# jlvdb/yet_another_wizz

Hardware: AMD Instinct MI355X
Metric: candidate pairs/s (higher is better)
Workload: dtype f64

## Files before the change

yet_another_wizz_amd/csrc/yawhip.hip:

```cpp

#include <hip/hip_runtime.h>

#include <algorithm>
#include <atomic>
#include <numeric>
#include <thread>
#include <chrono>
#include <climits>
#include <cmath>
#include <cstdarg>
#include <cstdio>
#include <cstdlib>
#include <cstring>
#include <memory>
#include <new>
#include <string>
#include <system_error>
#include <type_traits>
#include <utility>
#include <functional>
#include <vector>

#include "yawhip.h"
#include "yawhip_random.h"
// ... 202 lines not shown
    for (int d = -2; d <= 2; ++d) {
        const int64_t m = r + d;
        int64_t cnt = 0;
        if (d == 0) {
            cnt = i - off[r];
        } else if (m >= g_lo && m < g_hi) {
            int64_t l = off[m], h = off[m + 1];
            const int64_t base = l;
            if (d < 0) { while (l < h) { const int64_t mid = (l + h) >> 1; if (key[mid] <= ki) l = mid + 1; else h = mid; } }
            else       { while (l < h) { const int64_t mid = (l + h) >> 1; if (key[mid] < ki) l = mid + 1; else h = mid; } }
            cnt = l - base;
        }
        before[d + 2] = cnt;
    }
#pragma unroll
    for (int d = -1; d <= 1; ++d) {
        const int64_t t = r + d + 1 + 2 * g;
        const int64_t dst = off3[t] + before[d + 1] + before[d + 2] + before[d + 3];
        q3[dst] = fx; q3[q3_stride + dst] = fy; q3[2 * q3_stride + dst] = fz;
        idx3[dst] = (int32_t)i;
        if (w3) w3[dst] = wi;
        if (d == 0) pos3[i] = (int32_t)dst;
    }
}

constexpr int EVAL_SLOTS = 256;
constexpr int BUILD_WG = 1024;
constexpr int BUILD_WG_SMALL = 256;
inline int build_wg_for(int64_t n_pot) { return n_pot / 256 <= 4096 ? BUILD_WG_SMALL : BUILD_WG; }
constexpr int BUILD_PREFIX_LDS = 1024;

constexpr int ITEM_SEGS = 8;
__host__ __device__ constexpr int ITEM_SEG_CTR(int seg) { return 12 + 8 * seg; }
__device__ __forceinline__ void append_items(bool keep, const Item &it, unsigned long long work, Item *__restrict__ items,
                                             unsigned long long *__restrict__ counters, unsigned char *__restrict__ kept,
                                             unsigned long long seg_cap = 0) {
    if (keep && kept) kept[it.pot] = 1;
    __shared__ unsigned int s_cnt[BUILD_WG / 64];
    __shared__ unsigned long long s_work[BUILD_WG / 64], s_base;
    const unsigned long long mask = __builtin_amdgcn_ballot_w64(keep);
    const int lane = threadIdx.x & 63, wave = threadIdx.x >> 6;
    for (int off = 32; off > 0; off >>= 1) work += __shfl_down(work, off, 64);
    if (lane == 0) {
        s_cnt[wave] = (unsigned int)__popcll(mask);
        s_work[wave] = work;
    }
    __syncthreads();
    if (threadIdx.x == 0) {
        unsigned int total = 0;
        unsigned long long wsum = 0;
        for (int wv = 0; wv < (int)(blockDim.x >> 6); ++wv) {
            const unsigned int c = s_cnt[wv];
            s_cnt[wv] = total;
            total += c;
            wsum += s_work[wv];
        }
        if (seg_cap) {
            const int seg = (int)(blockIdx.x % ITEM_SEGS);
            s_base = (unsigned long long)seg * seg_cap + (total ? atomicAdd(&counters[ITEM_SEG_CTR(seg)], (unsigned long long)total) : 0ull);
        } else {
            s_base = total ? atomicAdd(&counters[0], (unsigned long long)total) : 0ull;
        }
        if (wsum) atomicAdd(&counters[10 + 8 * (blockIdx.x & (EVAL_SLOTS - 1))], wsum);
    }
    __syncthreads();
    if (keep) items[s_base + s_cnt[wave] + __popcll(mask & ((1ull << lane) - 1ull))] = it;
}

template <bool SWEEP>
__global__ __launch_bounds__(BUILD_WG) void k_build_items(CatView c1, CatView c2, const int32_t *__restrict__ jobs,
                                                     const int64_t *__restrict__ prefix, int n_slots, int n_bins,
                                                     int tile, const double *__restrict__ rwin, int64_t n_pot,
                                                     Item *__restrict__ items, unsigned long long *__restrict__ counters,
                                                     unsigned char *__restrict__ kept) {
    const int64_t pot = (int64_t)blockIdx.x * blockDim.x + threadIdx.x;
    bool keep = false;
    Item it{};
    unsigned long long work = 0;
    if (pot < n_pot) {
        int lo = 0, hi = n_slots;
        while (hi - lo > 1) {
            const int mid = (lo + hi) >> 1;
            if (prefix[mid] <= pot) lo = mid; else hi = mid;
        }
        const int slot = lo, job = slot / n_bins, k = slot - job * n_bins;
        const int p = jobs[2 * job], q = jobs[2 * job + 1];
        const int k1 = c1.nb == 1 ? 0 : k, k2 = c2.nb == 1 ? 0 : k;
        int64_t b0 = c1.off[(int64_t)p * c1.nb + k1], b1 = c1.off[(int64_t)p * c1.nb + k1 + 1];
        const int64_t a_seg1 = c2.off[(int64_t)q * c2.nb + k2 + 1];
        const int64_t a0 = c2.off[(int64_t)q * c2.nb + k2] + (pot - prefix[slot]) * (int64_t)tile;
        const int64_t a1 = a0 + tile < a_seg1 ? a0 + tile : a_seg1;
        if (SWEEP) {
            const double wlo = c2.key[a0] - rwin[k], whi = c2.key[a1 - 1] + rwin[k];
            int64_t l = b0, h = b1;
            while (l < h) {
                const int64_t m = (l + h) >> 1;
                if (c1.key[m] < wlo) l = m + 1; else h = m;
            }
            const int64_t first = l;
            h = b1;
            while (l < h) {
                const int64_t m = (l + h) >> 1;
                if (c1.key[m] <= whi) l = m + 1; else h = m;
            }
            b0 = first;
            b1 = l;
        }
        keep = b1 > b0;
        it.a0 = a0; it.b0[0] = b0; it.na = (int32_t)(a1 - a0); it.nb[0] = (int32_t)(b1 - b0); it.nwin = 1; it.slot = slot; it.pot = (int32_t)pot;
        work = keep ? (unsigned long long)it.na * (unsigned long long)it.nb[0] : 0ull;
    }
    if (SWEEP) {
        append_items(keep, it, work, items, counters, kept);
    } else {
        if (pot < n_pot) items[pot] = it;
        append_items(false, it, work, items, counters, nullptr);
        if (pot == 0) counters[0] = (unsigned long long)n_pot;
    }
}

__global__ __launch_bounds__(BUILD_WG) void k_build_items_strips(const DevTab *__restrict__ tabs, const JobRec *__restrict__ jobs,
                                                            const int64_t *__restrict__ prefix, int n_jobs, int reach,
                                                            int tile, double rwin, double cap_c, double cap_s, int swap,
                                                            int triple, int64_t n_pot,
                                                            Item *__restrict__ items, unsigned long long *__restrict__ counters,
                                                            unsigned char *__restrict__ kept, unsigned long long seg_cap) {
    const int64_t pot = (int64_t)blockIdx.x * blockDim.x + threadIdx.x;
    bool keep = false;
    Item it{};
    unsigned long long work = 0;
    __shared__ int64_t s_prefix[BUILD_PREFIX_LDS];
    __shared__ DevTab s_tabs[6];
    static_assert(sizeof(DevTab) % 8 == 0, "DevTab is copied in 8-byte words");
    for (int e = threadIdx.x; e < (int)(6 * sizeof(DevTab) / 8); e += blockDim.x)
        reinterpret_cast<uint64_t *>(s_tabs)[e] = reinterpret_cast<const uint64_t *>(tabs)[e];
    const bool prefix_in_lds = n_jobs + 1 <= BUILD_PREFIX_LDS;
    if (prefix_in_lds)
        for (int e = threadIdx.x; e <= n_jobs; e += blockDim.x) s_prefix[e] = prefix[e];
    __syncthreads();
    if (pot < n_pot) {
        int lo = 0, hi = n_jobs;
        if (prefix_in_lds) {
            while (hi - lo > 1) {
                const int mid = (lo + hi) >> 1;
                if (s_prefix[mid] <= pot) lo = mid; else hi = mid;
            }
        } else {
            while (hi - lo > 1) {
                const int mid = (lo + hi) >> 1;
                if (prefix[mid] <= pot) lo = mid; else hi = mid;
            }
        }
        const int job = lo;
        const JobRec jr = jobs[job];
        const int o = jr.o & 3;
        it.pad_ = (jr.o >> 2) & 1;
        const DevTab &c1 = s_tabs[swap ? 3 + o : o], &c2 = s_tabs[swap ? o : 3 + o];
        const gf64p key1d = tab_key(c1), key2 = tab_key(c2);
        const gf32p key1f = c1.axis == 0 ? c1.qx : (c1.axis == 1 ? c1.qy : c1.qz);
// ... 1270 lines not shown
                    (void)__hip_atomic_fetch_add((__attribute__((address_space(3))) unsigned int *)(size_t)pend[r], 1u,
                                                 __ATOMIC_RELAXED, __HIP_MEMORY_SCOPE_WORKGROUP);
            }
            if (!WEIGHTED && (stage_no & flush_mask) == flush_mask) flush_counts();
        }
        }
        if constexpr (WEIGHTED) {
            __syncthreads();
            for (int idx = lane; idx < nslots; idx += 64) {
                partials[(int64_t)it.pot * nslots + idx] = (double)hist[idx];
                hist[idx] = HistT(0);
            }
        } else {
            flush_counts();
        }
        nev = wave_sum_lane63(nev);
        if (lane == 63 && nev) atomicAdd(&counters[8 + 8 * (ticket & (EVAL_SLOTS - 1))], (unsigned long long)nev);
    }
}

__global__ void k_item_work(const Item *__restrict__ items, const unsigned long long *__restrict__ counters,
                            int slots_per_job, unsigned long long *__restrict__ job_work) {
    const unsigned long long i = (unsigned long long)blockIdx.x * blockDim.x + threadIdx.x;
    if (i >= counters[0]) return;
    const Item it = items[i];
    unsigned long long streamed = 0;
    for (int w = 0; w < it.nwin; ++w) streamed += (unsigned long long)it.nb[w];
    atomicAdd(&job_work[item_slot(it) / slots_per_job], (unsigned long long)it.na * streamed);
}

constexpr int REDUCE_CHUNK = 32;
__global__ void k_reduce_chunks(const double *__restrict__ partials, const unsigned char *__restrict__ kept,
                                const int64_t *__restrict__ prefix, const int64_t *__restrict__ cprefix, int n_slots,
                                int slab, double *__restrict__ chunk_sums) {
    const int64_t idx = (int64_t)blockIdx.x * blockDim.x + threadIdx.x;
    const int64_t g = idx / slab;
    if (g >= cprefix[n_slots]) return;
    const int e = (int)(idx - g * slab);
    int lo = 0, hi = n_slots;
    while (hi - lo > 1) {
        const int mid = (lo + hi) >> 1;
        if (cprefix[mid] <= g) lo = mid; else hi = mid;
    }
    const int64_t p0 = prefix[lo] + (g - cprefix[lo]) * REDUCE_CHUNK;
    const int64_t p1 = p0 + REDUCE_CHUNK < prefix[lo + 1] ? p0 + REDUCE_CHUNK : prefix[lo + 1];
    double acc = 0.0;
    for (int64_t pot = p0; pot < p1; ++pot)
        if (!kept || kept[pot]) acc += partials[pot * slab + e];
    chunk_sums[idx] = acc;
}

__global__ void k_reduce_slots(const double *__restrict__ chunk_sums, const int64_t *__restrict__ cprefix, int n_slots,
                               int slab, double *__restrict__ out) {
    const int64_t idx = (int64_t)blockIdx.x * blockDim.x + threadIdx.x;
    if (idx >= (int64_t)n_slots * slab) return;
    const int slot = (int)(idx / slab), e = (int)(idx - (int64_t)slot * slab);
    double acc = 0.0;
    for (int64_t g = cprefix[slot]; g < cprefix[slot + 1]; ++g) acc += chunk_sums[g * slab + e];
    out[idx] = acc;
}

template <typename F>
__device__ double numpy_sum_dev(F v, int lo, int n) {
    if (n < 8) {
        double res = 0.0;
        for (int i = 0; i < n; ++i) res += v(lo + i);
        return res;
    }
    if (n <= 128) {
        double r[8];
        for (int j = 0; j < 8; ++j) r[j] = v(lo + j);
        int i = 8;
        for (; i < n - (n % 8); i += 8)
            for (int j = 0; j < 8; ++j) r[j] += v(lo + i + j);
        double res = ((r[0] + r[1]) + (r[2] + r[3])) + ((r[4] + r[5]) + (r[6] + r[7]));
        for (; i < n; ++i) res += v(lo + i);
        return res;
    }
    int n2 = n / 2;
    n2 -= n2 % 8;
    return numpy_sum_dev(v, lo, n2) + numpy_sum_dev(v, lo + n2, n - n2);
}

__global__ void k_combine_scales(const unsigned long long *__restrict__ counts, const double *__restrict__ sums, int weighted,
                                 int64_t n_jobs, int n_bins, int nf, int n_scales, const int32_t *__restrict__ slices,
                                 const double *__restrict__ factors, double *__restrict__ out) {
    const int64_t i = (int64_t)blockIdx.x * blockDim.x + threadIdx.x;
    if (i >= n_jobs * n_bins * n_scales) return;
    const int sc = (int)(i % n_scales), k = (int)((i / n_scales) % n_bins);
    const int64_t j = i / ((int64_t)n_scales * n_bins);
    const int lo = slices[2 * (k * n_scales + sc)], hi = slices[2 * (k * n_scales + sc) + 1];
    const int64_t base = (j * n_bins + k) * (int64_t)nf;
    const double *wk = factors ? factors + (int64_t)k * nf : nullptr;
    auto value = [&](int e) {
        const double v = weighted ? sums[base + e] : (double)counts[base + e];
        return wk ? v * wk[e] : v;
    };
    out[i] = hi > lo ? numpy_sum_dev(value, lo, hi - lo) : 0.0;
}

__global__ void k_scatter_rows(const double *__restrict__ in, const int32_t *__restrict__ row_index, int64_t row, int64_t n,
                               double *__restrict__ out) {
    const int64_t i = (int64_t)blockIdx.x * blockDim.x + threadIdx.x;
    if (i >= n) return;
    const int64_t r = i / row;
    out[(int64_t)row_index[r] * row + (i - r * row)] = in[i];
}

__global__ void k_counts_to_double(const unsigned long long *__restrict__ in, double *__restrict__ out, int64_t n) {
    const int64_t i = (int64_t)blockIdx.x * blockDim.x + threadIdx.x;
    if (i < n) out[i] = (double)in[i];
}

inline DevTab make_tab(const double *x, const double *y, const double *z, const double *w, const int32_t *k, const int64_t *off,
                       const int64_t *vbase, const int64_t *slo, const int64_t *tiles, const TileRec *tile_rec, const RunGrid *grid,
                       int axis, const float *q = nullptr, int64_t q_stride = 0, const int32_t *idx = nullptr) {
    return DevTab{(gf64p)x, (gf64p)y, (gf64p)z, (gf64p)w, (gi32p)k, (gi64p)off, (gi64p)vbase, (gi64p)slo, (gi64p)tiles,
                  tile_rec, grid, (gf32p)q, (gf32p)(q ? q + q_stride : nullptr), (gf32p)(q ? q + 2 * q_stride : nullptr), (gi32p)idx,
                  (gi32p)nullptr, axis, 0};
}

template <typename T>
struct DevBuf {
    T *ptr = nullptr;
    size_t cap = 0;
    hipError_t reserve(size_t n) {
        if (n <= cap) return hipSuccess;
        if (ptr) (void)hipFree(ptr);
        ptr = nullptr;
        cap = 0;
        size_t want = n + n / 4 + 64;
        hipError_t e = hipMalloc(reinterpret_cast<void **>(&ptr), want * sizeof(T));
        if (e == hipSuccess) cap = want;
        return e;
    }
    void release() {
        if (ptr) (void)hipFree(ptr);
        ptr = nullptr;
        cap = 0;
    }
};

struct Arena {
    unsigned char *h = nullptr, *d = nullptr;
    size_t cap = 0;
    hipError_t reserve(size_t n) {
        if (n <= cap) return hipSuccess;
        release();
        const size_t want = n + n / 4 + 4096;
        hipError_t e = hipHostMalloc(reinterpret_cast<void **>(&h), want, hipHostMallocPortable);
        if (e == hipSuccess) e = hipMalloc(reinterpret_cast<void **>(&d), want);
        if (e == hipSuccess) cap = want; else release();
        return e;
    }
    void release() {
        if (h) (void)hipHostFree(h);
        if (d) (void)hipFree(d);
        h = d = nullptr;
        cap = 0;
    }
};
inline size_t align16(size_t n) { return (n + 15) & ~(size_t)15; }

}

struct CallBufs {
    hipEvent_t ev0 = nullptr, ev1 = nullptr, evc0 = nullptr, evc1 = nullptr, ev_done = nullptr;
    DevBuf<Item> d_items;
    unsigned long long *d_ctr = nullptr, *d_counts = nullptr;
    double *d_sums = nullptr;
    DevBuf<double> d_partials;
    DevBuf<double> d_chunk_sums;
    DevBuf<unsigned char> d_kept;
    Arena out;
    Arena comb;
    hipError_t make_events() {
        hipError_t e = hipSuccess;
        for (hipEvent_t *ev : {&ev0, &ev1, &evc0, &evc1, &ev_done})
            if (e == hipSuccess && !*ev) e = hipEventCreate(ev);
        return e;
    }
    void release_all() {
        d_items.release(); d_partials.release(); d_chunk_sums.release(); d_kept.release();
        out.release(); comb.release();
        for (hipEvent_t *ev : {&ev0, &ev1, &evc0, &evc1, &ev_done}) {
            if (*ev) (void)hipEventDestroy(*ev);
            *ev = nullptr;
        }
    }
};
constexpr int MAX_BATCH = 4;
constexpr size_t MAX_PLANS = 16;

namespace {
struct HostPlan;

struct CallKey {
    uint64_t c1_uid = 0, c2_uid = 0, opt_gen = 0, hash = 0;
    int32_t n_jobs = 0, n_bins = 0, n_edges = 0, kernel = 0, n_dev = 0;
    bool want_counts = false, want_sums = false, for_work = false;
    const int32_t *jobs = nullptr;
    const double *t = nullptr;
    std::vector<int32_t> own_jobs;
    std::vector<double> own_t;

    CallKey() = default;
    CallKey(const yawhip_ctx *ctx, const yawhip_catalog *c1, const yawhip_catalog *c2, int32_t n_jobs, const int32_t *jobs,
// ... 943 lines not shown
    if (c->x) (void)hipFree(c->x);
    if (c->y) (void)hipFree(c->y);
    if (c->z) (void)hipFree(c->z);
    if (c->w) (void)hipFree(c->w);
    if (c->off) (void)hipFree(c->off);
    for (int o = 0; o < 3; ++o) {
        c->strips[o].release();
        c->seg[o].release();
    }
    delete c;
    return YAWHIP_OK;
}

int yawhip_catalog_device_bytes(const yawhip_catalog *cat, int64_t *bytes) {
    if (!cat || !bytes) return fail(YAWHIP_ERR_INVALID, "yawhip_catalog_device_bytes: NULL argument");
    *bytes = cat->device_bytes;
    return YAWHIP_OK;
}

}

namespace {

struct CallState {
    std::chrono::steady_clock::time_point wall0;
    bool pending = false;
    int64_t n_out = 0;
    size_t o_ctr = 0, o_counts = 0, o_sums = 0;
    bool want_counts = false, want_sums = false, band_ran = false, run_unweighted = false, run_weighted = false;
    bool segmented = false;
    int64_t cand = 0, abytes = 0, n_pot = 0;
    int launches = 0, kernel = 0, mode = 0, n_orient = 0, band_variant = 0, merged_triples = 0;
    int32_t variant[2] = {0, 0};
};

enum VariantFamily : int32_t { VF_COUNT = 1, VF_MERGED, VF_MERGED_OCC8, VF_BAND, VF_BAND32, VF_BAND32_ONE, VF_BAND32_FINE };
constexpr int32_t variant_code(int32_t family, int R, int cap, bool weighted, int ne = 0, bool merged = false, bool uni = false,
                               bool priv = false, bool filter = false, bool nf1 = false) {
    return family | R << 4 | cap << 8 | (int32_t)weighted << 18 | ne << 19 | (int32_t)merged << 22 | (int32_t)uni << 23 |
           (int32_t)priv << 24 | (int32_t)filter << 25 | (int32_t)nf1 << 26;
}
int32_t merge_variant(int32_t a, int32_t b) { return a == 0 || a == b ? b : (b == 0 ? a : YAWHIP_VARIANT_MIXED); }

std::vector<float> build_thr32(const double *t, int n_bins, int n_edges) {
    auto down = [](double v) { float f = (float)v; if ((double)f > v) f = nextafterf(f, -INFINITY); return f; };
    auto up = [](double v) { float f = (float)v; if ((double)f < v) f = nextafterf(f, INFINITY); return f; };
    auto guard = [](double te) { return BAND32_GUARD_SQRT * std::sqrt(te) + 5e-7 * te + 1e-12; };
    const int tw = thr32_width(n_edges);
    std::vector<float> out((size_t)n_bins * tw, 0.f);
    for (int k = 0; k < n_bins; ++k) {
        const double *tk = t + (size_t)k * n_edges;
        float *row = &out[(size_t)k * tw];
        if (n_edges == 2) {
            const double g0 = guard(tk[0]), g1 = guard(tk[1]);
            const float c = (float)(0.5 * (tk[0] + tk[1]));
            const double cd = (double)c;
            const double fold = 4e-7 * cd;
            const double h_in = (std::min(cd - (tk[0] + g0), (tk[1] - g1) - cd) - fold) * (1.0 - 1e-6);
            const double h_out = (std::max(cd - (tk[0] - g0), (tk[1] + g1) - cd) + fold) * (1.0 + 1e-6);
            row[0] = c;
            row[1] = h_in > 0.0 ? down(h_in) : 0.f;
            row[2] = up(std::max(h_out, 0.0));
            row[3] = 0.f;
        } else {
            for (int e = 0; e < n_edges; ++e) {
                const double g = guard(tk[e]);
// ... 571 lines not shown
        if (cand_plan->key == key) {
            plan = cand_plan;
            break;
        }
    if (!plan) {
        std::unique_ptr<HostPlan> fresh(new (std::nothrow) HostPlan());
        if (!fresh) return fail(YAWHIP_ERR_OOM, "host allocation failed");
        const int rc = make_plan(ctx, c1, c2, n_jobs, jobs, n_bins, n_edges, t, kernel, want_counts, want_sums, job_work != nullptr, *fresh);
        if (rc != YAWHIP_OK) return rc;
        key.keep();
        fresh->key = std::move(key);
        if (ctx->plans.size() >= MAX_PLANS) {
            size_t old = 0;
            for (size_t i = 1; i < ctx->plans.size(); ++i)
                if (ctx->plans[i]->stamp < ctx->plans[old]->stamp) old = i;
            HIP_TRY(hipStreamSynchronize(ctx->stream));
            delete ctx->plans[old];
            ctx->plans[old] = ctx->plans.back();
            ctx->plans.pop_back();
        }
        plan = fresh.release();
        ctx->plans.push_back(plan);
    }
    plan->stamp = ++ctx->plan_clock;
    const HostPlan &P = *plan;
    cs.n_out = P.n_out;
    if (P.empty) return YAWHIP_OK;
    if (P.split) return SPLIT_JOBS;
    if (P.run_weighted) HIP_TRY(ctx->d_partials.reserve((size_t)std::max<int64_t>(P.n_items, 1) * P.slab));
    g_trace.mark("plan");
    const size_t o_ctr = 0, o_counts = align16(N_CTR * sizeof(unsigned long long)),
                 o_sums = o_counts + align16((size_t)P.n_out * sizeof(unsigned long long));
    const size_t out_bytes = o_sums + align16((size_t)P.n_out * sizeof(double));
    HIP_TRY(ctx->out.reserve(out_bytes));
    ctx->d_ctr = reinterpret_cast<unsigned long long *>(ctx->out.d + o_ctr);
    ctx->d_counts = reinterpret_cast<unsigned long long *>(ctx->out.d + o_counts);
    ctx->d_sums = reinterpret_cast<double *>(ctx->out.d + o_sums);
    HIP_TRY(hipMemsetAsync(ctx->out.d, 0, P.n_items > 0 ? o_sums : out_bytes, ctx->stream));

    int launches = 0;
    const int64_t n_pot = P.n_items;
    int64_t n_items = P.n_items;
    unsigned long long seg_cap = 0;
    g_trace.mark("memset");
    HIP_TRY(hipEventRecord(ctx->ev0, ctx->stream));
    if (n_pot > 0) {
        if (n_pot >= (1ll << 31))
            return fail(YAWHIP_ERR_INVALID, "too many work items (%lld) in one job", (long long)n_pot);
        const int bwg = build_wg_for(n_pot);
        const unsigned bgrid = (unsigned)((n_pot + bwg - 1) / bwg);
        if (P.strip_items && (P.band32 || P.band_fine) && !job_work && ctx->item_segments)
            seg_cap = (unsigned long long)((bgrid + ITEM_SEGS - 1) / ITEM_SEGS) * (unsigned long long)bwg;
        HIP_TRY(ctx->d_items.reserve(seg_cap ? (size_t)(seg_cap * ITEM_SEGS) : (size_t)n_pot));
        unsigned char *kept_flags = nullptr;
        if (P.run_weighted && P.sweep) {
            HIP_TRY(ctx->d_kept.reserve((size_t)n_pot));
            HIP_TRY(hipMemsetAsync(ctx->d_kept.ptr, 0, (size_t)n_pot, ctx->stream));
            kept_flags = ctx->d_kept.ptr;
        }
        if (P.strip_items)
            hipLaunchKernelGGL(k_build_items_strips, dim3(bgrid), dim3(bwg), 0, ctx->stream, P.d_tabs,
                               reinterpret_cast<const JobRec *>(P.d_jobs), P.d_prefix, (int)P.n_sjobs,
                               P.triple ? 0 : P.reach, (int)P.tile, P.rwin_max, P.cap_c, P.cap_s, P.swap ? 1 : 0, P.triple ? 1 : 0,
                               n_pot, ctx->d_items.ptr,
                               ctx->d_ctr, kept_flags, seg_cap);
        else if (P.sweep)
            hipLaunchKernelGGL(k_build_items<true>, dim3(bgrid), dim3(bwg), 0, ctx->stream, view_of(c1), view_of(c2),
                               P.d_jobs, P.d_prefix, (int)P.n_pslots, n_bins, (int)P.tile,
                               P.d_rwin, n_pot, ctx->d_items.ptr, ctx->d_ctr, kept_flags);
        else
            hipLaunchKernelGGL(k_build_items<false>, dim3(bgrid), dim3(bwg), 0, ctx->stream, view_of(c1), view_of(c2),
                               P.d_jobs, P.d_prefix, (int)P.n_pslots, n_bins, (int)P.tile, P.d_rwin, n_pot,
                               ctx->d_items.ptr, ctx->d_ctr, nullptr);
        HIP_TRY(hipGetLastError());
        ++launches;
        n_items = n_pot;
        if (P.strip_items && !P.band && n_pot > SYNC_GRID_MIN_ITEMS) {
            HIP_TRY(hipMemcpyAsync(ctx->out.h, ctx->d_ctr, 2 * sizeof(unsigned long long), hipMemcpyDeviceToHost, ctx->stream));
            HIP_TRY(hipStreamSynchronize(ctx->stream));
            n_items = (int64_t)reinterpret_cast<unsigned long long *>(ctx->out.h)[0];
        }
    }
    if (job_work) {
        HIP_TRY(ctx->d_jobwork.reserve((size_t)n_jobs));
        HIP_TRY(hipMemsetAsync(ctx->d_jobwork.ptr, 0, sizeof(unsigned long long) * (size_t)n_jobs, ctx->stream));
        if (n_pot > 0) {
            hipLaunchKernelGGL(k_item_work, dim3((unsigned)((n_pot + 255) / 256)), dim3(256), 0, ctx->stream, ctx->d_items.ptr,
                               ctx->d_ctr, P.merged ? 1 : n_bins, ctx->d_jobwork.ptr);
            HIP_TRY(hipGetLastError());
        }
        HIP_TRY(hipMemcpyAsync(job_work, ctx->d_jobwork.ptr, sizeof(int64_t) * (size_t)n_jobs, hipMemcpyDeviceToHost,
                               ctx->stream));
        HIP_TRY(hipStreamSynchronize(ctx->stream));
        return YAWHIP_OK;
    }
    auto reduce_partials = [&]() -> hipError_t {
        const int64_t n_oslots = P.n_pslots, values = P.slab, n_chunks = P.n_chunks;
        hipError_t er = ctx->d_chunk_sums.reserve((size_t)std::max<int64_t>(n_chunks, 1) * values);
        if (er != hipSuccess) return er;
        const int thr = 256;
        const bool all_kept = !(P.run_weighted && P.sweep);
        if (n_chunks > 0)
            hipLaunchKernelGGL(k_reduce_chunks, dim3((unsigned)((n_chunks * values + thr - 1) / thr)), dim3(thr), 0, ctx->stream,
                               ctx->d_partials.ptr, all_kept ? nullptr : ctx->d_kept.ptr, P.d_prefix, P.d_cprefix,
                               (int)n_oslots, (int)values, ctx->d_chunk_sums.ptr);
        hipLaunchKernelGGL(k_reduce_slots, dim3((unsigned)((n_oslots * values + thr - 1) / thr)), dim3(thr), 0, ctx->stream,
                           ctx->d_chunk_sums.ptr, P.d_cprefix, (int)n_oslots, (int)values, ctx->d_sums);
        return hipGetLastError();
    };
    HIP_TRY(hipEventRecord(ctx->evc0, ctx->stream));
    int64_t grid = P.strip_items && n_pot > 65536 ? n_pot / P.grid_div : n_pot;
    const int batch_log2 = ctx->band_batch_log2 >= 0 ? ctx->band_batch_log2 : 0;
    if (!P.run_weighted) grid = std::max<int64_t>(grid >> batch_log2, 8);
    grid = std::min<int64_t>((grid + 7) & ~7ll, 1ll << 22);
    const dim3 band_grid((unsigned)grid), wave(64);
    int flush_log2 = ctx->flush_log2;
    while (flush_log2 > 0 && ((uint64_t)64 * P.R * 2 * P.cap << flush_log2) >= (1ull << 32)) --flush_log2;
    const unsigned flush_mask = (1u << flush_log2) - 1u;
    const std::pair<int, int> stage{P.R, P.cap};
    const std::pair<bool, bool> rows{P.merged, P.uni};
    auto launch_band32 = [&](bool wgt) -> hipError_t {
        const size_t lds = band32_lds(P.weighted, P.cap, P.lean_bins * P.nf, P.merged && !P.uniform_t ? n_bins : 0, n_edges);
        const bool one_chunk = P.triple || !P.strip_items;
        return pick<Bool<false>, Bool<true>>(wgt, [&](auto w) {
            return pick<Int<4>, Int<3>, Int<2>>(n_edges, [&](auto ne) {
                return pick<Rows<true, false>, Rows<true, true>, Rows<false, true>>(rows, [&](auto r) {
                    return pick<Stage<4, B32_CAP_BIG>, Stage<2, B32_CAP_BIG>, Stage<2, B32_CAP>, Stage<1, B32_CAP>>(stage, [&](auto s) {
                        using S = decltype(s);
                        using M = decltype(r);
                        auto kern = one_chunk ? k_count_band32_one<S::R, S::CAP, w, ne, M::MERGED, M::UNI>
                                              : k_count_band32<S::R, S::CAP, w, ne, M::MERGED, M::UNI>;
                        cs.variant[w] = variant_code(one_chunk ? VF_BAND32_ONE : VF_BAND32, S::R, S::CAP, w, ne, M::MERGED, M::UNI);
                        return launch(kern, band_grid, wave, lds, ctx->stream, P.d_tabs, ctx->d_items.ptr, n_bins, P.d_t,
                                      P.d_thr32, P.d_rwin, P.d_ucap, flush_mask, P.swap ? 1 : 0, ctx->d_counts,
                                      ctx->d_partials.ptr, ctx->d_ctr, seg_cap);
                    });
                });
            });
        });
    };
    auto launch_band64 = [&](bool wgt) -> hipError_t {
        return pick<Bool<false>, Bool<true>>(wgt, [&](auto w) {
            return pick<Int<0>, Int<4>, Int<3>, Int<2>>(P.band_ne, [&](auto ne) {
// ... 54 lines not shown
    auto lds_for = [&](bool w, bool priv) { return lds_fixed + (size_t)P.nf * (priv ? WG : 1) * (w ? 8 : 4); };
    auto launch_plain = [&](bool wgt) -> hipError_t {
        const bool priv = lds_for(wgt, true) <= (size_t)ctx->lds_limit;
        return pick<Bool<true>, Bool<false>>(wgt, [&](auto w) {
            return pick<Bool<false>, Bool<true>>(priv, [&](auto pv) {
                return pick<Bool<false>, Bool<true>>(P.filter, [&](auto f) {
                    return pick<Int<4>, Int<2>, Int<1>>(P.R, [&](auto r) {
                        cs.variant[w] = variant_code(VF_COUNT, r, 0, w, 0, false, false, pv, f);
                        return in_pieces(WG, [&](dim3 g, int64_t base) {
                            return launch(k_count<r, w, pv, f>, g, dim3(WG), lds_for(w, pv), ctx->stream, view_of(c1), view_of(c2),
                                          ctx->d_items.ptr, n_bins, n_edges, P.d_t, P.d_dthr, base, ctx->d_counts,
                                          ctx->d_partials.ptr, ctx->d_ctr);
                        });
                    });
                });
            });
        });
    };
    const bool band_ran = n_items > 0 && P.lean && P.band;
    auto launch_count = [&](bool wgt) {
        if (band_ran) return P.band32 ? launch_band32(wgt) : (P.band_fine ? launch_fine(wgt) : launch_band64(wgt));
        return P.lean ? launch_lean(wgt) : launch_plain(wgt);
    };
    if (n_items > 0 && P.run_unweighted) {
        HIP_TRY(launch_count(false));
        ++launches;
    }
    if (n_items > 0 && P.run_weighted) {
        HIP_TRY(launch_count(true));
        ++launches;
        HIP_TRY(reduce_partials());
        launches += 2;
    }
    HIP_TRY(hipEventRecord(ctx->evc1, ctx->stream));
    if (!P.weighted && want_sums) {
        const int thr = 256;
        hipLaunchKernelGGL(k_counts_to_double, dim3((unsigned)((P.n_out + thr - 1) / thr)), dim3(thr), 0, ctx->stream,
                           ctx->d_counts, ctx->d_sums, P.n_out);
        HIP_TRY(hipGetLastError());
        ++launches;
    }
    HIP_TRY(hipEventRecord(ctx->ev1, ctx->stream));
    const size_t fetch = !fetch_results ? o_counts : (want_sums ? out_bytes : (want_counts ? o_sums : o_counts));
    HIP_TRY(hipMemcpyAsync(ctx->out.h, ctx->out.d, fetch, hipMemcpyDeviceToHost, ctx->stream));
    cs.pending = true;
    cs.o_ctr = o_ctr; cs.o_counts = o_counts; cs.o_sums = o_sums;
    cs.band_ran = band_ran; cs.run_unweighted = P.run_unweighted; cs.run_weighted = P.run_weighted;
    cs.cand = P.cand; cs.abytes = P.abytes; cs.n_pot = n_pot; cs.segmented = seg_cap != 0;
    cs.launches = launches; cs.kernel = P.kernel; cs.mode = P.mode;
    cs.n_orient = P.n_orient;
    cs.band_variant = !band_ran ? 0 : (P.band32 ? 32 : (P.band_fine ? 33 : 64));
    cs.merged_triples = band_ran && P.triple ? 1 : 0;
    g_trace.mark("launched");
    return YAWHIP_OK;
}

template <typename T>
void place_rows(T *out, const T *in, int64_t n_rows, int64_t row, const int32_t *at = nullptr) {
    if (!out) return;
    if (!at) {
        row *= n_rows;
        n_rows = 1;
    }
    for (int64_t r = 0; r < n_rows; ++r) {
        T *dst = out + (size_t)(at ? at[r] : 0) * (size_t)row;
        if (in) memcpy(dst, in + (size_t)r * row, sizeof(T) * (size_t)row);
        else memset(dst, 0, sizeof(T) * (size_t)row);
    }
}

int count_finish(yawhip_ctx *ctx, const CallState &cs, int64_t *fine_counts, double *fine_sums, yawhip_stats *stats,
                 const int32_t *row_index = nullptr, int64_t row_len = 0, bool wait_done = false) {
    if (stats) memset(stats, 0, sizeof *stats);
    const int64_t n_rows = !row_index ? 1 : (row_len > 0 ? cs.n_out / row_len : 0), row = row_index ? row_len : cs.n_out;
    if (!cs.pending) {
        place_rows<int64_t>(fine_counts, nullptr, n_rows, row, row_index);
        place_rows<double>(fine_sums, nullptr, n_rows, row, row_index);
        return YAWHIP_OK;
    }
    g_trace.mark("meanwhile");
    HIP_TRY(hipSetDevice(ctx->device));
    if (ctx->spin_wait) {
        hipError_t qe;
        const auto spin0 = std::chrono::steady_clock::now();
        while ((qe = wait_done ? hipEventQuery(ctx->ev_done) : hipStreamQuery(ctx->stream)) == hipErrorNotReady &&
               std::chrono::steady_clock::now() - spin0 < std::chrono::milliseconds(2))
            __builtin_ia32_pause();
        if (qe == hipErrorNotReady) qe = wait_done ? hipEventSynchronize(ctx->ev_done) : hipStreamSynchronize(ctx->stream);
        HIP_TRY(qe);
    } else {
        HIP_TRY(wait_done ? hipEventSynchronize(ctx->ev_done) : hipStreamSynchronize(ctx->stream));
    }
    g_trace.mark("waited");
    place_rows(fine_counts, reinterpret_cast<const int64_t *>(ctx->out.h + cs.o_counts), n_rows, row, row_index);
    place_rows(fine_sums, reinterpret_cast<const double *>(ctx->out.h + cs.o_sums), n_rows, row, row_index);
    const unsigned long long *ctr = reinterpret_cast<const unsigned long long *>(ctx->out.h + cs.o_ctr);
    g_trace.mark("copied");
    if (stats) {
        float ms = 0.f;
        HIP_TRY(hipEventElapsedTime(&ms, ctx->ev0, ctx->ev1));
        float cms = 0.f;
        HIP_TRY(hipEventElapsedTime(&cms, ctx->evc0, ctx->evc1));
        stats->count_ms = cms;
        stats->candidate_pairs = cs.cand;
        unsigned long long tile_pairs = 0;
        for (int i = 0; i < EVAL_SLOTS; ++i) tile_pairs += ctr[10 + 8 * (size_t)i];
        stats->evaluated_pairs = (int64_t)tile_pairs * ((cs.run_unweighted ? 1 : 0) + (cs.run_weighted ? 1 : 0));
        if (cs.band_ran) {
            unsigned long long ev = 0;
            for (int i = 0; i < EVAL_SLOTS; ++i) ev += ctr[8 + 8 * (size_t)i];
            stats->evaluated_pairs = (int64_t)ev;
        }
        stats->algorithmic_bytes = cs.abytes;
        stats->n_workgroups = cs.n_pot > 0 ? (int64_t)ctr[0] : 0;
        if (cs.segmented && cs.n_pot > 0)
            for (int sg = 0; sg < ITEM_SEGS; ++sg) stats->n_workgroups += (int64_t)ctr[ITEM_SEG_CTR(sg)];
        stats->n_launches = cs.launches;
        stats->kernel_used = cs.kernel;
        stats->layout_mode = cs.mode;
        stats->n_orientations = cs.n_orient;
        stats->band_variant = cs.band_variant;
        stats->merged_triples = cs.merged_triples;
        stats->count_variant = cs.variant[0];
        stats->count_variant_weighted = cs.variant[1];
        if (cs.band_ran)
            for (int i = 0; i < EVAL_SLOTS; ++i) stats->exact_reevaluations += (int64_t)ctr[9 + 8 * (size_t)i];
        stats->kernel_ms = ms;
        stats->total_ms = std::chrono::duration<double, std::milli>(std::chrono::steady_clock::now() - cs.wall0).count();
    }
    g_trace.mark("stats");
    return YAWHIP_OK;
}

void add_stats(yawhip_stats &total, const yawhip_stats &part, bool side_by_side) {
    total.candidate_pairs += part.candidate_pairs;
// ... 182 lines not shown
}

int yawhip_count_pairs_rows_device(yawhip_ctx *ctx, const yawhip_catalog *c1, const yawhip_catalog *c2, int32_t n_jobs,
                                   const int32_t *jobs, int32_t n_bins, int32_t n_edges, const double *t, int32_t kernel,
                                   int64_t n_rows_total, const int32_t *row_index, double **device_rows, yawhip_stats *stats) {
    if (stats) memset(stats, 0, sizeof *stats);
    if (!ctx || !c1 || !c2 || !device_rows) return fail(YAWHIP_ERR_INVALID, "yawhip_count_pairs_rows_device: NULL argument");
    *device_rows = nullptr;
    if (!ctx->peers.empty()) return fail(YAWHIP_ERR_INVALID, "yawhip_count_pairs_rows_device: single-device contexts only");
    const int rc_args = check_call(ctx, c1, c2, n_jobs, jobs, n_bins, n_edges, t);
    if (rc_args != YAWHIP_OK) return rc_args;
    if (n_rows_total < n_jobs || (n_jobs > 0 && !row_index))
        return fail(YAWHIP_ERR_INVALID, "yawhip_count_pairs_rows_device: bad sizes or NULL arrays");
    const int64_t row = (int64_t)n_bins * (n_edges - 1);
    for (int j = 0; j < n_jobs; ++j)
        if (row_index[j] < 0 || row_index[j] >= n_rows_total)
            return fail(YAWHIP_ERR_INVALID, "yawhip_count_pairs_rows_device: row index %d outside [0, %lld)", row_index[j], (long long)n_rows_total);
    HIP_TRY(hipSetDevice(ctx->device));
    const size_t n_full = (size_t)n_rows_total * (size_t)row + 1;
    HIP_TRY(ctx->d_full.reserve(n_full));
    HIP_TRY(ctx->d_rowidx.reserve((size_t)std::max(n_jobs, 1)));
    CallState cs;
    int rc = count_enqueue(ctx, c1, c2, n_jobs, jobs, n_bins, n_edges, t, kernel, false, true, nullptr, cs, false);
    if (rc == SPLIT_JOBS) {
        std::vector<double> rows((size_t)n_jobs * (size_t)row), full(n_full, 0.0);
        rc = run_single(ctx, c1, c2, n_jobs, jobs, n_bins, n_edges, t, kernel, nullptr, rows.data(), stats);
        if (rc != YAWHIP_OK) return rc;
        place_rows(full.data(), (const double *)rows.data(), n_jobs, row, row_index);
        HIP_TRY(hipMemcpy(ctx->d_full.ptr, full.data(), sizeof(double) * n_full, hipMemcpyHostToDevice));
        *device_rows = ctx->d_full.ptr;
        return YAWHIP_OK;
    }
    if (rc != YAWHIP_OK) return rc;
    HIP_TRY(hipMemsetAsync(ctx->d_full.ptr, 0, sizeof(double) * n_full, ctx->stream));
    if (cs.pending && n_jobs > 0) {
        HIP_TRY(hipMemcpyAsync(ctx->d_rowidx.ptr, row_index, sizeof(int32_t) * (size_t)n_jobs, hipMemcpyHostToDevice, ctx->stream));
        const int64_t n = (int64_t)n_jobs * row;
        hipLaunchKernelGGL(k_scatter_rows, dim3((unsigned)((n + 255) / 256)), dim3(256), 0, ctx->stream, ctx->d_sums,
                           ctx->d_rowidx.ptr, row, n, ctx->d_full.ptr);
        HIP_TRY(hipGetLastError());
    }
    rc = count_finish(ctx, cs, nullptr, nullptr, stats);
    if (rc != YAWHIP_OK) return rc;
    *device_rows = ctx->d_full.ptr;
    return YAWHIP_OK;
}

}

namespace {
double numpy_sum(const double *a, int64_t n) {
    if (n < 8) {
        double res = 0.0;
        for (int64_t i = 0; i < n; ++i) res += a[i];
        return res;
    }
    if (n <= 128) {
        double r[8];
        for (int j = 0; j < 8; ++j) r[j] = a[j];
        int64_t i = 8;
        for (; i < n - (n % 8); i += 8)
            for (int j = 0; j < 8; ++j) r[j] += a[i + j];
        double res = ((r[0] + r[1]) + (r[2] + r[3])) + ((r[4] + r[5]) + (r[6] + r[7]));
        for (; i < n; ++i) res += a[i];
        return res;
    }
// ... 16 lines not shown
}

namespace {

struct DenseState {
    CallState cs;
    bool enqueued = false;
    bool device_combine = false;
    bool weighted = false;
    int slot = 0;
    int64_t n_comb = 0;
    size_t h_comb_off = 0;
};

int dense_check(const yawhip_ctx *ctx, const yawhip_dense_request &r, int32_t n_bins, int32_t n_edges, const double *t,
                int32_t n_scales, const int32_t *slices) {
    const int rc = check_call(ctx, r.c1, r.c2, r.n_jobs, r.jobs, n_bins, n_edges, t);
    if (rc != YAWHIP_OK) return rc;
    if (n_scales <= 0 || !slices || !r.dense) return fail(YAWHIP_ERR_INVALID, "yawhip_count_pairs_dense: bad sizes or NULL arrays");
    return YAWHIP_OK;
}

int dense_enqueue(yawhip_ctx *ctx, const yawhip_dense_request &r, int32_t n_bins, int32_t n_edges, const double *t, int32_t kernel,
                  int32_t n_scales, const int32_t *slices, const double *fine_factors, DenseState &ds) {
    const int nf = n_edges - 1;
    ds.weighted = r.c1->w != nullptr || r.c2->w != nullptr;
    ds.slot = ctx->slot;
    ds.device_combine = nf > 1;
    int rc = count_enqueue(ctx, r.c1, r.c2, r.n_jobs, r.jobs, n_bins, n_edges, t, kernel, !ds.weighted, ds.weighted, nullptr, ds.cs,
                           !ds.device_combine);
    if (rc == SPLIT_JOBS) return YAWHIP_OK;
    if (rc != YAWHIP_OK) return rc;
    if (ds.device_combine) {
        ds.n_comb = (int64_t)r.n_jobs * n_bins * n_scales;
        const size_t b_slices = align16(sizeof(int32_t) * 2 * (size_t)n_bins * n_scales);
        const size_t b_fact = fine_factors ? align16(sizeof(double) * (size_t)n_bins * nf) : 0;
        HIP_TRY(ctx->comb.reserve(b_slices + b_fact + sizeof(double) * (size_t)std::max<int64_t>(ds.n_comb, 1)));
        memcpy(ctx->comb.h, slices, sizeof(int32_t) * 2 * (size_t)n_bins * n_scales);
        if (fine_factors) memcpy(ctx->comb.h + b_slices, fine_factors, sizeof(double) * (size_t)n_bins * nf);
        HIP_TRY(hipMemcpyAsync(ctx->comb.d, ctx->comb.h, b_slices + b_fact, hipMemcpyHostToDevice, ctx->stream));
        ds.h_comb_off = b_slices + b_fact;
        double *d_comb = reinterpret_cast<double *>(ctx->comb.d + ds.h_comb_off);
        if (ds.cs.pending && ds.n_comb > 0) {
            hipLaunchKernelGGL(k_combine_scales, dim3((unsigned)((ds.n_comb + 255) / 256)), dim3(256), 0, ctx->stream,
                               ctx->d_counts, ctx->d_sums, ds.weighted ? 1 : 0, (int64_t)r.n_jobs, n_bins, nf, n_scales,
                               reinterpret_cast<const int32_t *>(ctx->comb.d),
                               fine_factors ? reinterpret_cast<const double *>(ctx->comb.d + b_slices) : nullptr, d_comb);
            HIP_TRY(hipGetLastError());
            HIP_TRY(hipMemcpyAsync(ctx->comb.h + ds.h_comb_off, d_comb, sizeof(double) * (size_t)ds.n_comb, hipMemcpyDeviceToHost, ctx->stream));
        }
    }
    HIP_TRY(hipEventRecord(ctx->ev_done, ctx->stream));
    ds.enqueued = true;
    return YAWHIP_OK;
}

void dense_clear(const yawhip_dense_request &r, int32_t n_bins, int32_t n_scales) {
    const size_t P = (size_t)r.c1->n_patches;
    memset(r.dense, 0, sizeof(double) * (size_t)n_scales * (size_t)n_bins * P * P);
}

void dense_scatter(const yawhip_dense_request &r, int32_t n_bins, int32_t n_scales, const int32_t *slices, const double *fine_factors,
                   const double *comb, bool weighted, const int64_t *hc, const double *hs) {
    const int64_t P = r.c1->n_patches;
    const int32_t n_jobs = r.n_jobs;
    const int32_t *jobs = r.jobs;
// ... 334 lines not shown
```

Measured before the change: 29280000 billion.

## Replace result memcpy and events with device tail kernel writing coherent host memory

Replaces the device-to-host memcpy and timing events with a tail kernel that copies the result block straight into coherent pinned host memory, zeroes the counter block for the next call, and publishes a sequence word the host spins on. Timing now comes from device wall-clock stamps instead of events. Memsets are skipped when the block is already clean from the previous call's tail. This is meant to cut per-call launch, memset and copy overhead and the event-based host wait, at the cost of coherent-memory writes from the GPU and more complex state tracking.

```diff
diff --git a/yet_another_wizz_amd/csrc/yawhip.hip b/yet_another_wizz_amd/csrc/yawhip.hip
--- a/yet_another_wizz_amd/csrc/yawhip.hip
+++ b/yet_another_wizz_amd/csrc/yawhip.hip
@@ -258,6 +258,12 @@
 
 constexpr int ITEM_SEGS = 8;
 __host__ __device__ constexpr int ITEM_SEG_CTR(int seg) { return 12 + 8 * seg; }
+constexpr int CTR_T_BUILD = 1, CTR_T_COUNTED = 2, CTR_T_TAIL = 3, CTR_TICKET = 4, CTR_DONE = 6;
+__host__ __device__ constexpr int SEG_EXIT_CTR(int seg) { return ITEM_SEG_CTR(seg) + 1; }
+constexpr double CLOCK_MS = 1.0e-5;
+__device__ __forceinline__ void stamp_start(unsigned long long *__restrict__ counters, int word) {
+    if (blockIdx.x == 0 && threadIdx.x == 0) counters[word] = wall_clock64();
+}
 __device__ __forceinline__ void append_items(bool keep, const Item &it, unsigned long long work, Item *__restrict__ items,
                                              unsigned long long *__restrict__ counters, unsigned char *__restrict__ kept,
                                              unsigned long long seg_cap = 0) {
@@ -291,6 +297,7 @@
     }
     __syncthreads();
     if (keep) items[s_base + s_cnt[wave] + __popcll(mask & ((1ull << lane) - 1ull))] = it;
+    if (threadIdx.x == 0) atomicMax(&counters[SEG_EXIT_CTR((int)(blockIdx.x % ITEM_SEGS))], (unsigned long long)wall_clock64());
 }
 
 template <bool SWEEP>
@@ -299,6 +306,7 @@
                                                      int tile, const double *__restrict__ rwin, int64_t n_pot,
                                                      Item *__restrict__ items, unsigned long long *__restrict__ counters,
                                                      unsigned char *__restrict__ kept) {
+    stamp_start(counters, CTR_T_BUILD);
     const int64_t pot = (int64_t)blockIdx.x * blockDim.x + threadIdx.x;
     bool keep = false;
     Item it{};
@@ -351,6 +359,7 @@
                                                             int triple, int64_t n_pot,
                                                             Item *__restrict__ items, unsigned long long *__restrict__ counters,
                                                             unsigned char *__restrict__ kept, unsigned long long seg_cap) {
+    stamp_start(counters, CTR_T_BUILD);
     const int64_t pot = (int64_t)blockIdx.x * blockDim.x + threadIdx.x;
     bool keep = false;
     Item it{};
@@ -1687,7 +1696,8 @@
 constexpr int REDUCE_CHUNK = 32;
 __global__ void k_reduce_chunks(const double *__restrict__ partials, const unsigned char *__restrict__ kept,
                                 const int64_t *__restrict__ prefix, const int64_t *__restrict__ cprefix, int n_slots,
-                                int slab, double *__restrict__ chunk_sums) {
+                                int slab, double *__restrict__ chunk_sums, unsigned long long *__restrict__ counters) {
+    stamp_start(counters, CTR_T_COUNTED);
     const int64_t idx = (int64_t)blockIdx.x * blockDim.x + threadIdx.x;
     const int64_t g = idx / slab;
     if (g >= cprefix[n_slots]) return;
@@ -1706,7 +1716,8 @@
 }
 
 __global__ void k_reduce_slots(const double *__restrict__ chunk_sums, const int64_t *__restrict__ cprefix, int n_slots,
-                               int slab, double *__restrict__ out) {
+                               int slab, double *__restrict__ out, unsigned long long *__restrict__ stamp) {
+    if (stamp) stamp_start(stamp, CTR_T_COUNTED);
     const int64_t idx = (int64_t)blockIdx.x * blockDim.x + threadIdx.x;
     if (idx >= (int64_t)n_slots * slab) return;
     const int slot = (int)(idx / slab), e = (int)(idx - (int64_t)slot * slab);
@@ -1762,9 +1773,39 @@
     out[(int64_t)row_index[r] * row + (i - r * row)] = in[i];
 }
 
-__global__ void k_counts_to_double(const unsigned long long *__restrict__ in, double *__restrict__ out, int64_t n) {
+__global__ void k_counts_to_double(const unsigned long long *__restrict__ in, double *__restrict__ out, int64_t n,
+                                   unsigned long long *__restrict__ counters) {
+    stamp_start(counters, CTR_T_COUNTED);
     const int64_t i = (int64_t)blockIdx.x * blockDim.x + threadIdx.x;
     if (i < n) out[i] = (double)in[i];
+}
+
+constexpr int TAIL_WG = 256;
+constexpr unsigned TAIL_MAX_GRID = 64;
+__global__ __launch_bounds__(TAIL_WG) void k_call_tail(uint4 *__restrict__ dev, uint4 *__restrict__ host, unsigned n_copy,
+                                                      unsigned n_clean, unsigned long long seq) {
+    const unsigned long long t0 = wall_clock64();
+    static_assert(CTR_T_COUNTED == 2 && CTR_T_TAIL == 3 && CTR_TICKET == 4 && CTR_DONE == 6, "units 1, 2 and 3 of the block");
+    for (unsigned u = blockIdx.x * TAIL_WG + threadIdx.x; u < n_copy; u += gridDim.x * TAIL_WG) {
+        if (u == CTR_TICKET / 2 || u == CTR_DONE / 2) continue;
+        uint4 v = dev[u];
+        if (u == CTR_T_COUNTED / 2) {
+            if ((v.x | v.y) == 0u) { v.x = (unsigned)t0; v.y = (unsigned)(t0 >> 32); }
+            v.z = (unsigned)t0; v.w = (unsigned)(t0 >> 32);
+        }
+        host[u] = v;
+        if (u < n_clean) dev[u] = make_uint4(0u, 0u, 0u, 0u);
+    }
+    __threadfence_system();
+    __syncthreads();
+    if (threadIdx.x == 0) {
+        unsigned *ticket = reinterpret_cast<unsigned *>(dev) + 2 * CTR_TICKET;
+        if (atomicInc(ticket, gridDim.x - 1) == gridDim.x - 1) {
+            __threadfence_system();
+            __hip_atomic_store(reinterpret_cast<unsigned long long *>(host) + CTR_DONE, seq, __ATOMIC_RELEASE,
+                               __HIP_MEMORY_SCOPE_SYSTEM);
+        }
+    }
 }
 
 inline DevTab make_tab(const double *x, const double *y, const double *z, const double *w, const int32_t *k, const int64_t *off,
@@ -1803,7 +1844,7 @@
         if (n <= cap) return hipSuccess;
         release();
         const size_t want = n + n / 4 + 4096;
-        hipError_t e = hipHostMalloc(reinterpret_cast<void **>(&h), want, hipHostMallocPortable);
+        hipError_t e = hipHostMalloc(reinterpret_cast<void **>(&h), want, hipHostMallocPortable | hipHostMallocCoherent);
         if (e == hipSuccess) e = hipMalloc(reinterpret_cast<void **>(&d), want);
         if (e == hipSuccess) cap = want; else release();
         return e;
@@ -1828,6 +1869,9 @@
     DevBuf<double> d_chunk_sums;
     DevBuf<unsigned char> d_kept;
     Arena out;
+    bool dirty = true;
+    size_t zero_upto = 0;
+    uint64_t seq = 0;
     Arena comb;
     hipError_t make_events() {
         hipError_t e = hipSuccess;
@@ -2837,6 +2881,11 @@
     int64_t cand = 0, abytes = 0, n_pot = 0;
     int launches = 0, kernel = 0, mode = 0, n_orient = 0, band_variant = 0, merged_triples = 0;
     int32_t variant[2] = {0, 0};
+    uint64_t seq = 0;
+    bool word_wait = true;
+    bool stamps = false;
+    bool cleaned = false;
+    size_t zero_after = 0;
 };
 
 enum VariantFamily : int32_t { VF_COUNT = 1, VF_MERGED, VF_MERGED_OCC8, VF_BAND, VF_BAND32, VF_BAND32_ONE, VF_BAND32_FINE };
@@ -3474,18 +3523,31 @@
     const size_t o_ctr = 0, o_counts = align16(N_CTR * sizeof(unsigned long long)),
                  o_sums = o_counts + align16((size_t)P.n_out * sizeof(unsigned long long));
     const size_t out_bytes = o_sums + align16((size_t)P.n_out * sizeof(double));
+    const unsigned char *const block_was = ctx->out.d;
     HIP_TRY(ctx->out.reserve(out_bytes));
+    if (ctx->out.d != block_was) {
+        ctx->dirty = true;
+        reinterpret_cast<unsigned long long *>(ctx->out.h)[CTR_DONE] = 0;
+    }
     ctx->d_ctr = reinterpret_cast<unsigned long long *>(ctx->out.d + o_ctr);
     ctx->d_counts = reinterpret_cast<unsigned long long *>(ctx->out.d + o_counts);
     ctx->d_sums = reinterpret_cast<double *>(ctx->out.d + o_sums);
-    HIP_TRY(hipMemsetAsync(ctx->out.d, 0, P.n_items > 0 ? o_sums : out_bytes, ctx->stream));
+    const size_t zero_needed = P.n_items > 0 ? o_sums : out_bytes;
+    if (ctx->dirty) ctx->zero_upto = 0;
+    if (ctx->zero_upto < zero_needed) {
+        HIP_TRY(hipMemsetAsync(ctx->out.d + ctx->zero_upto, 0, zero_needed - ctx->zero_upto, ctx->stream));
+        ctx->zero_upto = zero_needed;
+    }
+    ctx->dirty = true;
+    cs.seq = ++ctx->seq;
+    cs.stamps = P.n_items > 0;
 
     int launches = 0;
     const int64_t n_pot = P.n_items;
     int64_t n_items = P.n_items;
     unsigned long long seg_cap = 0;
     g_trace.mark("memset");
-    HIP_TRY(hipEventRecord(ctx->ev0, ctx->stream));
+    if (!cs.stamps) HIP_TRY(hipEventRecord(ctx->ev0, ctx->stream));
     if (n_pot > 0) {
         if (n_pot >= (1ll << 31))
             return fail(YAWHIP_ERR_INVALID, "too many work items (%lld) in one job", (long long)n_pot);
@@ -3545,12 +3607,13 @@
         if (n_chunks > 0)
             hipLaunchKernelGGL(k_reduce_chunks, dim3((unsigned)((n_chunks * values + thr - 1) / thr)), dim3(thr), 0, ctx->stream,
                                ctx->d_partials.ptr, all_kept ? nullptr : ctx->d_kept.ptr, P.d_prefix, P.d_cprefix,
-                               (int)n_oslots, (int)values, ctx->d_chunk_sums.ptr);
+                               (int)n_oslots, (int)values, ctx->d_chunk_sums.ptr, ctx->d_ctr);
         hipLaunchKernelGGL(k_reduce_slots, dim3((unsigned)((n_oslots * values + thr - 1) / thr)), dim3(thr), 0, ctx->stream,
-                           ctx->d_chunk_sums.ptr, P.d_cprefix, (int)n_oslots, (int)values, ctx->d_sums);
+                           ctx->d_chunk_sums.ptr, P.d_cprefix, (int)n_oslots, (int)values, ctx->d_sums,
+                           n_chunks > 0 ? nullptr : ctx->d_ctr);
         return hipGetLastError();
     };
-    HIP_TRY(hipEventRecord(ctx->evc0, ctx->stream));
+    if (!cs.stamps) HIP_TRY(hipEventRecord(ctx->evc0, ctx->stream));
     int64_t grid = P.strip_items && n_pot > 65536 ? n_pot / P.grid_div : n_pot;
     const int batch_log2 = ctx->band_batch_log2 >= 0 ? ctx->band_batch_log2 : 0;
     if (!P.run_weighted) grid = std::max<int64_t>(grid >> batch_log2, 8);
@@ -3671,17 +3734,29 @@
         HIP_TRY(reduce_partials());
         launches += 2;
     }
-    HIP_TRY(hipEventRecord(ctx->evc1, ctx->stream));
+    if (!cs.stamps) HIP_TRY(hipEventRecord(ctx->evc1, ctx->stream));
     if (!P.weighted && want_sums) {
         const int thr = 256;
         hipLaunchKernelGGL(k_counts_to_double, dim3((unsigned)((P.n_out + thr - 1) / thr)), dim3(thr), 0, ctx->stream,
-                           ctx->d_counts, ctx->d_sums, P.n_out);
+                           ctx->d_counts, ctx->d_sums, P.n_out, ctx->d_ctr);
         HIP_TRY(hipGetLastError());
         ++launches;
     }
-    HIP_TRY(hipEventRecord(ctx->ev1, ctx->stream));
+    if (!cs.stamps) HIP_TRY(hipEventRecord(ctx->ev1, ctx->stream));
     const size_t fetch = !fetch_results ? o_counts : (want_sums ? out_bytes : (want_counts ? o_sums : o_counts));
-    HIP_TRY(hipMemcpyAsync(ctx->out.h, ctx->out.d, fetch, hipMemcpyDeviceToHost, ctx->stream));
+    const size_t clean = std::min(fetch, o_sums);
+    const bool sums_written = P.n_items > 0 && (P.run_weighted || want_sums);
+    cs.cleaned = clean == o_sums;
+    cs.zero_after = sums_written ? o_sums : ctx->zero_upto;
+    const unsigned n_copy = (unsigned)(fetch / 16), n_clean = (unsigned)(clean / 16);
+    static_assert(N_CTR * sizeof(unsigned long long) % 16 == 0 && (CTR_DONE + 2) * sizeof(unsigned long long) <= N_CTR * sizeof(unsigned long long),
+                  "the tail's words lie inside the counter block");
+    if (fetch / 16 > 0xffffffffull) return fail(YAWHIP_ERR_INVALID, "result block too large (%zu bytes)", fetch);
+    hipLaunchKernelGGL(k_call_tail, dim3(std::min((n_copy + TAIL_WG - 1) / TAIL_WG, TAIL_MAX_GRID)), dim3(TAIL_WG), 0, ctx->stream,
+                       reinterpret_cast<uint4 *>(ctx->out.d), reinterpret_cast<uint4 *>(ctx->out.h), n_copy, n_clean,
+                       (unsigned long long)cs.seq);
+    HIP_TRY(hipGetLastError());
+    ++launches;
     cs.pending = true;
     cs.o_ctr = o_ctr; cs.o_counts = o_counts; cs.o_sums = o_sums;
     cs.band_ran = band_ran; cs.run_unweighted = P.run_unweighted; cs.run_weighted = P.run_weighted;
@@ -3720,26 +3795,48 @@
     g_trace.mark("meanwhile");
     HIP_TRY(hipSetDevice(ctx->device));
     if (ctx->spin_wait) {
-        hipError_t qe;
+        const unsigned long long *done_word = reinterpret_cast<const unsigned long long *>(ctx->out.h) + CTR_DONE;
+        auto query = [&]() { return wait_done ? hipEventQuery(ctx->ev_done) : hipStreamQuery(ctx->stream); };
+        hipError_t qe = hipErrorNotReady;
         const auto spin0 = std::chrono::steady_clock::now();
-        while ((qe = wait_done ? hipEventQuery(ctx->ev_done) : hipStreamQuery(ctx->stream)) == hipErrorNotReady &&
-               std::chrono::steady_clock::now() - spin0 < std::chrono::milliseconds(2))
+        do {
+            if (cs.word_wait) {
+                if (__atomic_load_n(done_word, __ATOMIC_ACQUIRE) == cs.seq) qe = hipSuccess;
+            } else {
+                qe = query();
+            }
+            if (qe != hipErrorNotReady) break;
             __builtin_ia32_pause();
+        } while (std::chrono::steady_clock::now() - spin0 < std::chrono::milliseconds(2));
+        if (qe == hipSuccess && cs.word_wait) {
+            const hipError_t late = query();
+            if (late != hipErrorNotReady) qe = late;
+        }
         if (qe == hipErrorNotReady) qe = wait_done ? hipEventSynchronize(ctx->ev_done) : hipStreamSynchronize(ctx->stream);
         HIP_TRY(qe);
     } else {
         HIP_TRY(wait_done ? hipEventSynchronize(ctx->ev_done) : hipStreamSynchronize(ctx->stream));
     }
     g_trace.mark("waited");
+    if (cs.cleaned) {
+        ctx->dirty = false;
+        ctx->zero_upto = cs.zero_after;
+    }
     place_rows(fine_counts, reinterpret_cast<const int64_t *>(ctx->out.h + cs.o_counts), n_rows, row, row_index);
     place_rows(fine_sums, reinterpret_cast<const double *>(ctx->out.h + cs.o_sums), n_rows, row, row_index);
     const unsigned long long *ctr = reinterpret_cast<const unsigned long long *>(ctx->out.h + cs.o_ctr);
     g_trace.mark("copied");
     if (stats) {
-        float ms = 0.f;
-        HIP_TRY(hipEventElapsedTime(&ms, ctx->ev0, ctx->ev1));
-        float cms = 0.f;
-        HIP_TRY(hipEventElapsedTime(&cms, ctx->evc0, ctx->evc1));
+        float ms = 0.f, cms = 0.f;
+        if (cs.stamps) {
+            unsigned long long built = 0;
+            for (int sg = 0; sg < ITEM_SEGS; ++sg) built = std::max(built, ctr[SEG_EXIT_CTR(sg)]);
+            ms = (float)((double)(ctr[CTR_T_TAIL] - ctr[CTR_T_BUILD]) * CLOCK_MS);
+            cms = (float)((double)(ctr[CTR_T_COUNTED] - built) * CLOCK_MS);
+        } else {
+            HIP_TRY(hipEventElapsedTime(&ms, ctx->ev0, ctx->ev1));
+            HIP_TRY(hipEventElapsedTime(&cms, ctx->evc0, ctx->evc1));
+        }
         stats->count_ms = cms;
         stats->candidate_pairs = cs.cand;
         unsigned long long tile_pairs = 0;
@@ -3988,6 +4085,7 @@
         return YAWHIP_OK;
     }
     if (rc != YAWHIP_OK) return rc;
+    cs.word_wait = false;
     HIP_TRY(hipMemsetAsync(ctx->d_full.ptr, 0, sizeof(double) * n_full, ctx->stream));
     if (cs.pending && n_jobs > 0) {
         HIP_TRY(hipMemcpyAsync(ctx->d_rowidx.ptr, row_index, sizeof(int32_t) * (size_t)n_jobs, hipMemcpyHostToDevice, ctx->stream));
@@ -4070,6 +4168,7 @@
     if (rc == SPLIT_JOBS) return YAWHIP_OK;
     if (rc != YAWHIP_OK) return rc;
     if (ds.device_combine) {
+        ds.cs.word_wait = false;
         ds.n_comb = (int64_t)r.n_jobs * n_bins * n_scales;
         const size_t b_slices = align16(sizeof(int32_t) * 2 * (size_t)n_bins * n_scales);
         const size_t b_fact = fine_factors ? align16(sizeof(double) * (size_t)n_bins * nf) : 0;
```

After: 32380000 billion, median of 6. +10.6%, better.
